# jinryan/RangeCLIP

Hardware: NVIDIA B200
Metric: pixel_text_infonce_fwd_bwd_throughput (higher is better)
Workload: dtype bf16

## Files before the change

include/rangeclip_b200.h:

```cpp
#ifndef RANGECLIP_B200_H_
#define RANGECLIP_B200_H_

#include <stdint.h>

#ifdef __cplusplus
extern "C" {
#endif

#define RC_ABI_VERSION 1

typedef enum { RC_F32 = 0, RC_BF16 = 1 } rc_dtype;

typedef enum {
  RC_OK = 0,
  RC_ERR_INVALID = -1,
  RC_ERR_UNSUPPORTED = -2,
  RC_ERR_CUDA = -3,
  RC_ERR_NO_DEVICE = -4
} rc_status;

int rc_abi_version(void);
const char* rc_last_error(void);
int64_t rc_launch_count(void);


int64_t rc_infonce_workspace_bytes(int B, int D, int64_t HW, int K, rc_dtype x_dtype);
int64_t rc_infonce_workspace_bytes_dt(int B, int D, int64_t HW, int K, rc_dtype x_dtype);

int rc_infonce_f32(const float* x, int B, int D, int64_t HW, int64_t ld_b,
                   const float* t, int K, const int32_t* y, const float* w, float inv_tau,
                   float* lse, double* loss_sum, double* w_sum,
                   const double* w_sum_in, const float* grad_scale,
                   float* dx, float* dt, double* dlogtau, void* stream);

#define RC_INFONCE_PREPASS_DONE 1
#define RC_INFONCE_KEEP_WEIGHT 2
#define RC_INFONCE_LSE_GIVEN 4
#define RC_INFONCE_TS_KERNEL 8
#define RC_INFONCE_ACCUMULATE_DX 16
int rc_infonce_bf16(const void* x, rc_dtype x_dtype, int B, int D, int64_t HW,
                    const void* t_bf16, const void* tt_bf16, int K,
                    const int32_t* y, const float* w, float inv_tau,
                    float* lse, double* loss_sum, double* w_sum,
                    const double* w_sum_in, const float* grad_scale,
                    void* dx, float* dt, double* dlogtau,
                    void* workspace, int64_t workspace_bytes, int flags, void* stream);
int rc_infonce_bf16_rep4(const void* x, rc_dtype x_dtype, int B, int D, int64_t HW,
                         const void* t_bf16, const void* tt_bf16, int K,
                         const int32_t* y4, const float* w4, float inv_tau,
                         float* lse, double* loss_sum, double* w_sum,
                         const double* w_sum_in, const float* grad_scale,
                         void* dx, float* dt, double* dlogtau,
                         void* workspace, int64_t workspace_bytes, int flags, void* stream);
int rc_infonce_bf16_kblocks(const void* x, rc_dtype x_dtype, int D, int64_t HW,
                            const void* t_bf16_all, const void* tt_bf16_all, int K, int n_blocks,
                            const int32_t* y_rel, const float* w_rep, float inv_tau,
                            float* lse, double* loss_sum, double* w_sum, const double* w_sum_in, const float* grad_scale,
                            void* dx_blocks, double* dlogtau, void* workspace, int64_t workspace_bytes, int flags, void* stream);
int rc_infonce_bf16_dyn(const void* x, rc_dtype x_dtype, int B, int D, int64_t HW,
                        const void* t_bf16, const void* tt_bf16, int K, const int32_t* k_dev,
                        const int32_t* y, const float* w, const float* log_tau_dev, int rep,
// ... 87 lines not shown
```

rangeclip_b200/csrc/infonce_ts.cu:

```cuda
#include "common.cuh"
#include "umma.cuh"
#include <float.h>
#include <stdlib.h>

namespace rc {
using namespace umma;

namespace ts {

#ifndef RC_TS_X_HINT
#define RC_TS_X_HINT 0
#endif

constexpr int kTilePx = 128;
constexpr int kThreads = 640;
constexpr int kXStages = 6;
constexpr int kTStages = 3;
constexpr int kStageBytes = 16 * 1024;
constexpr int kEpiBufs = 4;
constexpr int kEpiAhead = 2;
constexpr int kEpiBufBytes = 2048;
constexpr int kTmemCols = 512;
constexpr int kSlotCols = 256;
constexpr int kColAcc = 128, kAccCols = 64;
constexpr int kRegsCtl = 48, kRegsSoftmax = 120;
constexpr float kLog2e = 1.4426950408889634f;
constexpr float kLn2 = 0.6931471805599453f;

struct __align__(8) Bars {
  uint64_t xf[kXStages];
  uint64_t xfull[kXStages], xempty[kXStages];
  uint64_t tfull[kTStages], tempty[kTStages];
  uint64_t s_full[2], p_full[2];
  uint64_t acc_full[2][2], acc_empty[2][2];
  uint64_t sc_full[4];
  uint64_t ebar[8][kEpiBufs];
  uint32_t tmem_base, pad;
};

constexpr int kScaleBufs = 4;
constexpr int kOffT = kXStages * kStageBytes;
constexpr int kOffEpi = kOffT + kTStages * kStageBytes;
constexpr int kOffScale = kOffEpi + 8 * kEpiBufs * kEpiBufBytes;
constexpr int kOffXch = kOffScale + kScaleBufs * 128 * 4;
constexpr int kOffPart = kOffXch + 2 * 4 * 2 * 128 * 4;
constexpr int kOffBars = kOffPart + 8 * 128 * 4;
constexpr int kSmemBytes = kOffBars + (int)sizeof(Bars);
static_assert(kSmemBytes <= 232448, "shared-memory budget of one SM (227 KB)");

struct Params {
  int B, D, K, Kp;
  int64_t HW;
  int tiles_per_img, n_tiles, n_pairs;
  uint32_t tpi_magic;
  int keep_w;
  int acc_dx;
  const float* lse_in;
  int kb;
  const int32_t* y;
  const float* w;
  float inv_tau;
  const float* grad_scale;
  const double* w_sum_in;
  float* lse;
  double* loss_sum;
  double* w_sum;
  double* dlogtau;
};

__device__ __forceinline__ int div_tiles(const Params& prm, int tile) {
  int q = (int)__umulhi((uint32_t)tile, prm.tpi_magic);
  if (tile - q * prm.tiles_per_img >= prm.tiles_per_img) ++q;
  return q;
// ... 47 lines not shown
  const int n_clusters = gridDim.x / 2;
  const int cluster_id = blockIdx.x / 2;
  const int my_pairs = cluster_id < prm.n_pairs ? (prm.n_pairs - cluster_id + n_clusters - 1) / n_clusters : 0;

  if (threadIdx.x == 0) {
    tma_prefetch_desc(&map_x_s); tma_prefetch_desc(&map_t); tma_prefetch_desc(&map_tt);
    tma_prefetch_desc(&map_xe); tma_prefetch_desc(&map_dx);
    for (int i = 0; i < kXStages; ++i) { mbar_init(&bars->xf[i], 1); mbar_init(&bars->xfull[i], 2); mbar_init(&bars->xempty[i], 9); }
    for (int i = 0; i < kTStages; ++i) { mbar_init(&bars->tfull[i], 1); mbar_init(&bars->tempty[i], 1); }
    for (int sl = 0; sl < 2; ++sl) {
      mbar_init(&bars->s_full[sl], 1); mbar_init(&bars->p_full[sl], 16);
      for (int ab = 0; ab < 2; ++ab) { mbar_init(&bars->acc_full[sl][ab], 1); mbar_init(&bars->acc_empty[sl][ab], 16); }
    }
    for (int i = 0; i < kScaleBufs; ++i) mbar_init(&bars->sc_full[i], 4);
    for (int i = 0; i < 8; ++i)
      for (int j = 0; j < kEpiBufs; ++j) mbar_init(&bars->ebar[i][j], 1);
    fence_barrier_init();
  }
  if (warp == 2) tmem_alloc_2sm<kTmemCols>(&bars->tmem_base);
  tc_fence_before();
  cluster_sync();
  tc_fence_after();
  const uint32_t tmem = bars->tmem_base;
  const uint32_t idesc_s = make_idesc_bf16(256, prm.Kp,  1,  0);
  const uint32_t idesc_d = make_idesc_bf16(256, kAccCols, 0, 0);
  auto arrive_leader = [&](uint64_t* bar) {
    if (leader_cta) mbar_arrive(bar);
    else mbar_arrive_remote(map_to_cta(bar, 0));
  };
  auto arrive_leader_warp = [&](uint64_t* bar) {
    __syncwarp();
    if (elect_one()) arrive_leader(bar);
  };
  auto pair_of = [&](int l) -> int { return cluster_id + l * n_clusters; };
  auto koff_of = [&](int pj) -> int { return (kKB && prm.kb > 0) ? div_tiles(prm, 2 * pj) * 256 : 0; };

  if (warp < 4) {
    asm volatile("setmaxnreg.dec.sync.aligned.u32 %0;" ::"n"(kRegsCtl));
    if (warp == 0 && lane == 0) {
      uint32_t it = 0;
      auto load_s = [&](int l) {
        const int koff = koff_of(pair_of(l));
        for (int c = 0; c < n_dchunks; ++c, ++it) {
          const int st = it % kTStages;
          mbar_wait(&bars->tempty[st], ((it / kTStages) & 1) ^ 1, 1);
          if (leader_cta) mbar_arrive_expect_tx(&bars->tfull[st], 2 * Nh * 128);
          tma_load_2d_2sm(smem + kOffT + st * kStageBytes, &map_t, &bars->tfull[st], c * 64, koff + (int)rank * Nh);
        }
      };
      auto load_dx = [&](int l) {
        const int koff = koff_of(pair_of(l));
        for (int blk = 0; blk < n_blk; ++blk, ++it) {
          const int st = it % kTStages;
          mbar_wait(&bars->tempty[st], ((it / kTStages) & 1) ^ 1, 2);
          if (leader_cta) mbar_arrive_expect_tx(&bars->tfull[st], 2 * n_kchunks * 4096);
          for (int kc = 0; kc < n_kchunks; ++kc)
            tma_load_2d_2sm(smem + kOffT + st * kStageBytes + kc * 4096, &map_tt, &bars->tfull[st], koff + kc * 64,
                            blk * 64 + (int)rank * 32);
        }
      };
      if (my_pairs > 0) load_s(0);
      if (my_pairs > 1) load_s(1);
      for (int l = 0; l < my_pairs; ++l) {
        load_dx(l);
        if (l + 2 < my_pairs) load_s(l + 2);
      }
    } else if (warp == 3 && lane == 0) {
      uint32_t xit = 0;
      const uint64_t pol_keep = RC_TS_X_HINT ? l2_policy_evict_last() : 0;
      for (int l = 0; l < my_pairs; ++l) {
        int b, px0;
        tile_coords(prm, 2 * pair_of(l) + (int)rank, b, px0);
        for (int c = 0; c < n_dchunks; ++c, ++xit) {
          const int st = xit % kXStages;
          mbar_wait(&bars->xempty[st], ((xit / kXStages) & 1) ^ 1, 3);
          uint8_t* sb = smem + st * kStageBytes;
          mbar_arrive_expect_tx(&bars->xf[st], 2 * 8192);
          const int bx = (kKB && prm.kb > 0) ? (b < prm.B ? 0 : 1) : b;
          if (RC_TS_X_HINT) {
            tma_load_3d_hint(sb, &map_x_s, &bars->xf[st], px0, c * 64, bx, pol_keep);
            tma_load_3d_hint(sb + 8192, &map_x_s, &bars->xf[st], px0 + 64, c * 64, bx, pol_keep);
          } else {
            tma_load_3d(sb, &map_x_s, &bars->xf[st], px0, c * 64, bx);
            tma_load_3d(sb + 8192, &map_x_s, &bars->xf[st], px0 + 64, c * 64, bx);
          }
        }
      }
    } else if (warp == 1 && leader_cta) {
      uint32_t it = 0, xit = 0;
      uint32_t acc_uses[2][2] = {{0, 0}, {0, 0}};
      const uint32_t smem_base = smem_u32(smem);
      const uint64_t dsc_x = desc_mnmajor_sw128(0, 8192);
      const uint64_t dsc_k = desc_kmajor_sw128(0);
      auto wait_acc_free = [&](int sl, int ab) {
        mbar_wait(&bars->acc_empty[sl][ab], (acc_uses[sl][ab] & 1u) ^ 1u, 7);
      };
      auto issue_s = [&](int l) {
        const int sl = l & 1;
        const uint32_t s_tmem = tmem + sl * kSlotCols;
        wait_acc_free(sl, 0);
        wait_acc_free(sl, 1);
        tc_fence_after();
        for (int c = 0; c < n_dchunks; ++c, ++it, ++xit) {
          const int sa = xit % kXStages, sb_ = it % kTStages;
          mbar_wait(&bars->xfull[sa], (xit / kXStages) & 1, 5);
          mbar_wait(&bars->tfull[sb_], (it / kTStages) & 1, 6);
          tc_fence_after();
          const uint64_t xa = dsc_x + ((smem_base + sa * kStageBytes) >> 4);
          const uint64_t tb = dsc_k + ((smem_base + kOffT + sb_ * kStageBytes) >> 4);
          if (elect_one()) {
#pragma unroll
            for (int ks = 0; ks < 4; ++ks)
              mma_bf16_ss_2sm(s_tmem, xa + ((ks * 2048) >> 4), tb + ((ks * 32) >> 4), idesc_s, (c | ks) != 0);
            mma_commit_2sm(&bars->xempty[sa]);
            mma_commit_2sm(&bars->tempty[sb_]);
            if (c + 1 == n_dchunks) mma_commit_2sm(&bars->s_full[sl]);
          }
          __syncwarp();
        }
      };
      auto issue_dx = [&](int l) {
        const int sl = l & 1;
        const uint32_t base = tmem + sl * kSlotCols;
        mbar_wait(&bars->p_full[sl], (l >> 1) & 1, 9);
        tc_fence_after();
        for (int blk = 0; blk < n_blk; ++blk, ++it) {
          const int ab = blk & 1;
          wait_acc_free(sl, ab);
          const int st = it % kTStages;
          mbar_wait(&bars->tfull[st], (it / kTStages) & 1, 8);
          tc_fence_after();
          const uint64_t sb = dsc_k + ((smem_base + kOffT + st * kStageBytes) >> 4);
          const uint32_t dcol = base + kColAcc + ab * kAccCols;
          if (elect_one()) {
            for (int kc = 0; kc < n_kchunks; ++kc) {
#pragma unroll
              for (int ks = 0; ks < 4; ++ks)
                mma_bf16_ts_2sm(dcol, base + (kc * 4 + ks) * 8, sb + ((kc * 4096 + ks * 32) >> 4), idesc_d, (kc | ks) != 0);
            }
            mma_commit_2sm(&bars->tempty[st]);
            mma_commit_2sm(&bars->acc_full[sl][ab]);
          }
          __syncwarp();
          ++acc_uses[sl][ab];
        }
      };
      if (my_pairs > 0) issue_s(0);
      if (my_pairs > 1) issue_s(1);
      for (int l = 0; l < my_pairs; ++l) {
        issue_dx(l);
        if (l + 2 < my_pairs) issue_s(l + 2);
      }
    } else if (warp == 2 && lane == 0) {
      uint32_t xit = 0;
      for (int l = 0; l < my_pairs; ++l)
        for (int c = 0; c < n_dchunks; ++c, ++xit) {
          const int st = xit % kXStages;
          mbar_wait(&bars->xf[st], (xit / kXStages) & 1, 10);
          arrive_leader(&bars->xfull[st]);
        }
    }
  } else if (warp < 12) {
    asm volatile("setmaxnreg.inc.sync.aligned.u32 %0;" ::"n"(kRegsSoftmax));
    const int half = warp >= 8 ? 1 : 0;
    const int row = (warp & 3) * 32 + lane;
    const int Kh = prm.Kp >> 1;
    const int cb = half * Kh;
    const uint32_t lane_base = tmem + ((uint32_t)((warp & 3) * 32) << 16);
    float* xch_base = reinterpret_cast<float*>(smem + kOffXch);
    float loss_acc = 0.f, w_acc = 0.f, dlt_acc = 0.f;
    float inv_wsum = 0.f, gscale = 1.f;
    {
      const double ws = prm.w_sum_in[0];
      inv_wsum = ws > 0.0 ? (float)(1.0 / ws) : 0.f;
      if (prm.grad_scale) gscale = prm.grad_scale[0];
    }
    float nx_ok = 0.f, nx_w = 0.f;
    int nx_y = -1;
    auto load_pixel_scalars = [&](int l) {
      nx_ok = 0.f; nx_w = 0.f; nx_y = -1;
      if (l >= my_pairs) return;
      const int t = 2 * pair_of(l) + (int)rank;
      if (t < prm.n_tiles) {
        const int tb = div_tiles(prm, t);
        const int tpx = (t - tb * prm.tiles_per_img) * kTilePx + row;
        if (tpx < prm.HW) {
          const int64_t tm = (int64_t)tb * prm.HW + tpx;
          nx_ok = 1.f;
          if (R == 1) {
            nx_y = __ldg(prm.y + tm);
            nx_w = __ldg(prm.w + tm);
          } else {
            const int4 y4 = __ldg(reinterpret_cast<const int4*>(prm.y) + tm);
            nx_y = (y4.x & 255) | ((y4.y & 255) << 8) | ((y4.z & 255) << 16) | ((y4.w & 255) << 24);
          }
        }
      }
    };
    load_pixel_scalars(0);
    float* part_s = reinterpret_cast<float*>(smem + kOffPart);
    const int st_ = threadIdx.x - 128;
    const int ng = st_ & 15, nr = st_ >> 4;
    uint32_t nit = 0;
    auto norm_tile = [&]() -> float {
      float ss[8];
#pragma unroll
      for (int j = 0; j < 8; ++j) ss[j] = 0.f;
      for (int c = 0; c < n_dchunks; ++c, ++nit) {
        const int st = nit % kXStages;
        mbar_wait(&bars->xf[st], (nit / kXStages) & 1, 11);
        const uint8_t* base = smem + st * kStageBytes + (ng >> 3) * 8192 + nr * 128;
        const int ch = ng & 7;
#pragma unroll
        for (int rr = 0; rr < 4; ++rr) {
          const int rowd = nr + rr * 16;
          const uint4 v = *reinterpret_cast<const uint4*>(base + rr * 2048 + ((ch ^ (rowd & 7)) << 4));
          const uint32_t u[4] = {v.x, v.y, v.z, v.w};
#pragma unroll
          for (int j = 0; j < 4; ++j) {
            ss[2 * j] = sqacc_bf16x2_lo(ss[2 * j], u[j]);
            ss[2 * j + 1] = sqacc_bf16x2_hi(ss[2 * j + 1], u[j]);
          }
        }
        __syncwarp();
        if (elect_one()) mbar_arrive(&bars->xempty[st]);
      }
#pragma unroll
      for (int j = 0; j < 8; ++j) ss[j] += __shfl_xor_sync(0xffffffffu, ss[j], 16);
      if (lane < 16) {
        float4* dst = reinterpret_cast<float4*>(part_s + (warp - 4) * 128 + ng * 8);
        dst[0] = make_float4(ss[0], ss[1], ss[2], ss[3]);
        dst[1] = make_float4(ss[4], ss[5], ss[6], ss[7]);
      }
      named_bar_sync(5, 256);
      float q = 0.f;
#pragma unroll
      for (int wv = 0; wv < 8; ++wv) q += part_s[wv * 128 + row];
      return 1.f / fmaxf(sqrtf(q), 1e-12f);
    };
    const bool use_bound = prm.inv_tau * (2.02f * kLog2e) < 100.f;
    const float ml_bound = prm.inv_tau * (1.01f * kLog2e);
    for (int l = 0; l < my_pairs; ++l) {
      const int sl = l & 1;
      const int tile = 2 * pair_of(l) + (int)rank;
      const bool tile_ok = tile < prm.n_tiles;
      const int b = tile_ok ? div_tiles(prm, tile) : 0;
      const int px = tile_ok ? (tile - b * prm.tiles_per_img) * kTilePx + row : 0;
      const bool valid = tile_ok && px < prm.HW;
      const int64_t m = (int64_t)b * prm.HW + px;
      const int Kt = (kKB && prm.kb > 0) ? min(256, prm.K - 256 * b) : prm.K;
      const bool px_ok = nx_ok != 0.f;
      const int yi = nx_y;
      const float wi = (R == 1 && (yi >= 0 || (kKB && prm.keep_w))) ? nx_w : 0.f;
      load_pixel_scalars(l + 1);
      float* xch = xch_base + (l & 1) * (4 * 2 * 128);
      const uint32_t trow = lane_base + sl * kSlotCols + cb;
      const float inv_n_tile = norm_tile();
      const float inv_n = px_ok ? inv_n_tile : 0.f;
      const float zs = inv_n * prm.inv_tau;
      const float zl = zs * kLog2e;
      mbar_wait(&bars->s_full[sl], (l >> 1) & 1, 12);
      tc_fence_after();
      float ml = ml_bound;
      if (!use_bound) {
        float mx = -FLT_MAX;
        for (int c = 0; c * 32 < Kh; ++c) {
          const int nvalid = Kt - (cb + c * 32);
          if (nvalid <= 0) break;
          uint32_t r[32];
          tmem_ld_32x32(trow + c * 32, r);
          tmem_ld_wait();
#pragma unroll
          for (int i = 0; i < 32; ++i) if (i < nvalid) mx = fmaxf(mx, __uint_as_float(r[i]));
        }
        xch[(0 * 2 + half) * 128 + row] = mx;
        named_bar_sync(3, 256);
        mx = fmaxf(mx, xch[(0 * 2 + (half ^ 1)) * 128 + row]);
        ml = mx * zl;
      }
      uint32_t pk[64];
      float s0 = 0.f, s1 = 0.f, s2 = 0.f, s3 = 0.f, q0 = 0.f, q1 = 0.f, q2 = 0.f, q3 = 0.f;
      float sy[R];
#pragma unroll
      for (int j = 0; j < R; ++j) sy[j] = 0.f;
#pragma unroll
// ... 43 lines not shown
      } else {
        int4 y4 = make_int4(-1, -1, -1, -1);
        float4 w4 = make_float4(0.f, 0.f, 0.f, 0.f);
        if (px_ok) {
          y4 = __ldg(reinterpret_cast<const int4*>(prm.y) + m);
          w4 = __ldg(reinterpret_cast<const float4*>(prm.w) + m);
        }
        const int ya[4] = {y4.x, y4.y, y4.z, y4.w};
        const float wa[4] = {w4.x, w4.y, w4.z, w4.w};
#pragma unroll
        for (int j = 0; j < R; ++j) { yj[j] = ya[j]; wj[j] = ya[j] >= 0 ? wa[j] : 0.f; }
      }
      float wtot = 0.f, tz = 0.f;
      bool mine[R];
#pragma unroll
      for (int j = 0; j < R; ++j) {
        mine[j] = yj[j] >= cb && yj[j] < cb + Kh;
        wtot += wj[j];
        tz += mine[j] ? wj[j] * sy[j] : 0.f;
      }
      xch[(1 * 2 + half) * 128 + row] = sum;
      xch[(2 * 2 + half) * 128 + row] = sez;
      xch[(3 * 2 + half) * 128 + row] = tz;
      tc_fence_before();
      named_bar_sync(2, 256);
      tc_fence_after();
      sum += xch[(1 * 2 + (half ^ 1)) * 128 + row];
      sez += xch[(2 * 2 + (half ^ 1)) * 128 + row];
      tz += xch[(3 * 2 + (half ^ 1)) * 128 + row];
      if (kKB && prm.lse_in != nullptr && valid) sum = fast_exp2(fmaf(__ldg(prm.lse_in + (prm.kb > 0 ? (int64_t)px : m)), kLog2e, -ml));
      float lse = 0.f;
      if (half == 0) {
        lse = (ml + __log2f(sum)) * kLn2;
        loss_acc += wtot * lse - tz * zs;
        w_acc += wtot;
      }
      const float coefb = gscale * inv_wsum;
      const float coef = coefb * wtot;
      const float inv_sum = 1.f / sum;
      const float rsv = inv_n * prm.inv_tau * coef * inv_sum;
      if (half == 0) {
        const float cj = coef * sez * zs * inv_sum - coefb * tz * zs;
        sc_s[(l & (kScaleBufs - 1)) * 128 + row] = -(inv_n * inv_n * cj);
        dlt_acc -= cj;
        __syncwarp();
        if (lane == 0) mbar_arrive(&bars->sc_full[l & (kScaleBufs - 1)]);
      }
      {
        const uint32_t prow = lane_base + sl * kSlotCols + (cb >> 1);
        const uint32_t rs2 = pack_bf16x2(rsv, rsv);
        uint32_t g16[R];
        int grel[R];
#pragma unroll
        for (int j = 0; j < R; ++j) {
          grel[j] = -1;
          g16[j] = 0;
          if (mine[j]) {
            const float ey = fast_exp2(fmaf(sy[j], zl, -ml));
            float gv;
            if (R == 1) {
              gv = (ey - sum) * rsv;
            } else {
              float wk = 0.f;
#pragma unroll
              for (int i = 0; i < R; ++i) wk += (yj[i] == yj[j]) ? wj[i] : 0.f;
              gv = (ey - sum * (wtot > 0.f ? wk / wtot : 0.f)) * rsv;
            }
// ... 4 lines not shown
#pragma unroll
        for (int c = 0; c < 4; ++c) {
          if (c * 32 < Kh) {
            uint32_t v[16];
#pragma unroll
            for (int i = 0; i < 16; ++i) v[i] = bf2_mul(pk[c * 16 + i], rs2);
#pragma unroll
            for (int j = 0; j < R; ++j) {
              if (grel[j] >= 0 && (grel[j] >> 5) == c) {
                const int jj = (grel[j] >> 1) & 15;
                const bool hi = grel[j] & 1;
#pragma unroll
                for (int i = 0; i < 16; ++i)
                  if (i == jj) v[i] = hi ? ((v[i] & 0xffffu) | (g16[j] << 16)) : ((v[i] & 0xffff0000u) | g16[j]);
              }
            }
            tmem_st_32x16(prow + c * 16, v);
          }
        }
        tmem_st_wait();
        tc_fence_before();
        arrive_leader_warp(&bars->p_full[sl]);
      }
      if (half == 0 && valid && prm.lse && !(kKB && prm.lse_in != nullptr)) prm.lse[m] = lse;
    }
    if (half == 0) {
      loss_acc = warp_sum(loss_acc); w_acc = warp_sum(w_acc); dlt_acc = warp_sum(dlt_acc);
      if (lane == 0) {
        if (prm.loss_sum) atomicAdd(prm.loss_sum, (double)loss_acc);
        if (prm.w_sum) atomicAdd(prm.w_sum, (double)w_acc);
        if (prm.dlogtau) atomicAdd(prm.dlogtau, (double)dlt_acc);
      }
    }
  } else {
    const int ew = warp - 12;
    const int q = warp & 3, h = ew >> 2;
    uint8_t* ebuf = smem + kOffEpi + ew * (kEpiBufs * kEpiBufBytes);
    uint64_t* ebar = &bars->ebar[ew][0];
    const int total = my_pairs * n_blk;
    const uint64_t pol_first = l2_policy_evict_first();
    struct Cursor { int l, u, px, bo, bx; };
    auto cursor_pair = [&](Cursor& cu) {
      int b, px0;
      tile_coords(prm, 2 * pair_of(cu.l) + (int)rank, b, px0);
      cu.px = px0 + q * 32;
      cu.bo = b;
      cu.bx = (kKB && prm.kb > 0) ? (b < prm.B ? 0 : 1) : b;
    };
    auto cursor_next = [&](Cursor& cu) {
      if (++cu.u == n_blk) { cu.u = 0; ++cu.l; cursor_pair(cu); }
    };
    Cursor cs{0, 0, 0, 0, 0}, cr{0, 0, 0, 0, 0};
    cursor_pair(cs);
    cursor_pair(cr);
    int s_req = 0;
    auto request_x = [&]() {
      const int bi = s_req % kEpiBufs;
      mbar_arrive_expect_tx(&ebar[bi], kEpiBufBytes);
      tma_load_3d(ebuf + bi * kEpiBufBytes, &map_xe, &ebar[bi], cr.px, cr.u * 64 + h * 32, cr.bx);
    };
    for (; s_req < kEpiAhead && s_req < total; ++s_req) {
      if (lane == 0) request_x();
      cursor_next(cr);
    }
    const uint32_t moff = (uint32_t)((lane & 7) * 64 + ((((lane >> 3) ^ ((lane >> 1) & 3)) & 3) << 4));
    int s = 0;
    uint32_t acc_seen[2][2] = {{0, 0}, {0, 0}};
    for (int l = 0; l < my_pairs; ++l) {
      const int sl = l & 1;
      mbar_wait(&bars->sc_full[l & (kScaleBufs - 1)], (l >> 2) & 1, 14);
      uint32_t ncs2[4];
#pragma unroll
      for (int pb = 0; pb < 4; ++pb) {
        const float v = sc_s[(l & (kScaleBufs - 1)) * 128 + q * 32 + pb * 8 + (lane >> 2)];
        ncs2[pb] = pack_bf16x2(v, v);
      }
      const uint32_t tacc = tmem + ((uint32_t)(q * 32) << 16) + sl * kSlotCols + kColAcc + h * 32;
      for (int blk = 0; blk < n_blk; ++blk, ++s) {
        const int ab = blk & 1;
        mbar_wait(&bars->acc_full[sl][ab], acc_seen[sl][ab] & 1u, 15);
        ++acc_seen[sl][ab];
        tc_fence_after();
        uint32_t pa[4][4];
        {
          uint32_t r[16];
          tmem_ld_16x256b_x4(tacc + ab * kAccCols, r);
          tmem_ld_wait();
#pragma unroll
          for (int g = 0; g < 4; ++g) {
            pa[g][0] = pack_bf16x2(__uint_as_float(r[4 * g]), __uint_as_float(r[4 * g + 1]));
            pa[g][1] = pack_bf16x2(__uint_as_float(r[4 * g + 2]), __uint_as_float(r[4 * g + 3]));
          }
          tmem_ld_16x256b_x4(tacc + ab * kAccCols + (16u << 16), r);
          tmem_ld_wait();
#pragma unroll
          for (int g = 0; g < 4; ++g) {
            pa[g][2] = pack_bf16x2(__uint_as_float(r[4 * g]), __uint_as_float(r[4 * g + 1]));
            pa[g][3] = pack_bf16x2(__uint_as_float(r[4 * g + 2]), __uint_as_float(r[4 * g + 3]));
          }
        }
        tc_fence_before();
        arrive_leader_warp(&bars->acc_empty[sl][ab]);
        const int bi = s % kEpiBufs;
        mbar_wait(&ebar[bi], (s / kEpiBufs) & 1, 16);
        const uint32_t bx0 = smem_u32(ebuf + bi * kEpiBufBytes) + moff;
        uint32_t xm[4][4];
#pragma unroll
        for (int g = 0; g < 4; ++g) ldmatrix_x4_trans(bx0 + g * 512, xm[g]);
#pragma unroll
        for (int g = 0; g < 4; ++g) {
#pragma unroll
          for (int pb = 0; pb < 4; ++pb) xm[g][pb] = bf2_fma(ncs2[pb], xm[g][pb], pa[g][pb]);
          stmatrix_x4_trans(bx0 + g * 512, xm[g]);
        }
        fence_proxy_async_smem();
        __syncwarp();
        if (lane == 0) {
          if (kKB && prm.acc_dx) tma_reduce_add_3d(&map_dx, ebuf + bi * kEpiBufBytes, cs.px, cs.u * 64 + h * 32, cs.bo);
          else tma_store_3d_hint(&map_dx, ebuf + bi * kEpiBufBytes, cs.px, cs.u * 64 + h * 32, cs.bo, pol_first);
          tma_store_commit();
          if (s_req < total) {
            asm volatile("cp.async.bulk.wait_group.read %0;" ::"n"(kEpiBufs - kEpiAhead) : "memory");
            request_x();
          }
        }
        cursor_next(cs);
        if (s_req < total) { cursor_next(cr); ++s_req; }
        __syncwarp();
      }
    }
    if (lane == 0) tma_store_wait_all0();
  }
  tc_fence_before();
  cluster_sync();
  if (warp == 2) {
    tc_fence_after();
    tmem_dealloc_2sm<kTmemCols>(tmem);
  }
}

}

int launch_infonce_ts(const void* xsrc, void* dx, const void* t_bf16, const void* tt_bf16, int B, int D, int64_t HW, int K,
                      const int32_t* y, const float* w, float inv_tau, const float* grad_scale, const double* w_sum_in,
                      float* lse, double* loss_sum, double* w_sum, double* dlogtau, int rep, int keep_w, const float* lse_in,
                      int kb, int acc_dx, cudaStream_t s) {
  using namespace ts;
  const int Kp = kb > 0 ? 256 : (K + 63) / 64 * 64;
  const int Kall = kb > 0 ? kb * 256 : Kp;
  CUtensorMap m_xs, m_t, m_tt, m_xe, m_dx;
  int rcode;
  {
    const uint64_t dims[3] = {(uint64_t)HW, (uint64_t)D, (uint64_t)B};
    const uint64_t xdims[3] = {(uint64_t)HW, (uint64_t)D, (uint64_t)(kb > 0 ? 1 : B)};
    const uint64_t str[3] = {2, (uint64_t)HW * 2, (uint64_t)D * HW * 2};
    const uint32_t box_s[3] = {64, 64, 1};
    if ((rcode = make_tmap_bf16(&m_xs, xsrc, 3, xdims, str, box_s, "ts map_x_s"))) return rcode;
    const uint32_t box_o[3] = {32, 32, 1};
    if ((rcode = make_tmap_bf16(&m_xe, xsrc, 3, xdims, str, box_o, "ts map_xe"))) return rcode;
    if ((rcode = make_tmap_bf16(&m_dx, dx, 3, dims, str, box_o, "ts map_dx"))) return rcode;
    const uint64_t tdims[2] = {(uint64_t)D, (uint64_t)Kall}, tstr[2] = {2, (uint64_t)D * 2};
    const uint32_t tbox[2] = {64, (uint32_t)(Kp / 2)};
    if ((rcode = make_tmap_bf16(&m_t, t_bf16, 2, tdims, tstr, tbox, "ts map_t"))) return rcode;
    const uint64_t ttdims[2] = {(uint64_t)Kall, (uint64_t)D}, ttstr[2] = {2, (uint64_t)Kall * 2};
    const uint32_t ttbox[2] = {64, 32};
    if ((rcode = make_tmap_bf16(&m_tt, tt_bf16, 2, ttdims, ttstr, ttbox, "ts map_tt"))) return rcode;
  }
  Params prm;
  prm.B = B; prm.D = D; prm.K = K; prm.Kp = Kp; prm.HW = HW;
  prm.tiles_per_img = (int)((HW + kTilePx - 1) / kTilePx);
  if ((int64_t)B * prm.tiles_per_img > 0x3fffffff) return fail(RC_ERR_UNSUPPORTED, "rc_infonce_bf16: too many tiles");
  prm.n_tiles = B * prm.tiles_per_img;
  prm.tpi_magic = prm.tiles_per_img == 1 ? 0xffffffffu : (uint32_t)(0x100000000ull / (uint64_t)prm.tiles_per_img);
  prm.n_pairs = (prm.n_tiles + 1) / 2;
  prm.y = y; prm.w = w; prm.inv_tau = inv_tau; prm.grad_scale = grad_scale;
  prm.w_sum_in = w_sum_in; prm.lse = lse; prm.loss_sum = loss_sum; prm.w_sum = w_sum; prm.dlogtau = dlogtau;
  prm.keep_w = keep_w; prm.lse_in = lse_in; prm.kb = kb; prm.acc_dx = acc_dx;
  if (kb > 0 && (prm.tiles_per_img & 1)) return fail(RC_ERR_UNSUPPORTED, "rc_infonce_bf16_kblocks: HW must be a multiple of 256");
  int n_clusters = num_sms() / 2;
  if (n_clusters > prm.n_pairs) n_clusters = prm.n_pairs;
  const int grid = 2 * n_clusters;
  auto launch = [&](auto kernel) -> int {
    cudaError_t e = cudaFuncSetAttribute(kernel, cudaFuncAttributeMaxDynamicSharedMemorySize, kSmemBytes);
    if (e != cudaSuccess) return fail(RC_ERR_CUDA, "rc_infonce_bf16(ts): smem opt-in: %s", cudaGetErrorString(e));
    kernel<<<grid, kThreads, kSmemBytes, s>>>(m_xs, m_t, m_tt, m_xe, m_dx, prm);
    return check_launch("rc_infonce_bf16(ts)");
  };
  if (rep == 4) return launch(infonce_ts_kernel<4, false>);
  if (keep_w || lse_in != nullptr || kb > 0 || acc_dx) return launch(infonce_ts_kernel<1, true>);
  return launch(infonce_ts_kernel<1, false>);
}
// ... 89 lines not shown
```

rangeclip_b200/csrc/infonce_umma.cu:

```cuda
#include "common.cuh"
#include "umma.cuh"
#include <float.h>
#include <stdlib.h>

namespace rc {

using namespace umma;

PFN_encodeTiled get_encode_tiled() {
  static PFN_encodeTiled fn = nullptr;
  static bool tried = false;
  if (!tried) {
    tried = true;
    void* p = nullptr;
    cudaDriverEntryPointQueryResult qres;
    if (cudaGetDriverEntryPoint("cuTensorMapEncodeTiled", &p, cudaEnableDefault, &qres) == cudaSuccess &&
        qres == cudaDriverEntryPointSuccess)
      fn = (PFN_encodeTiled)p;
  }
  return fn;
}

int make_tmap_bf16(CUtensorMap* out, const void* base, int rank, const uint64_t* dims, const uint64_t* strides_bytes,
                   const uint32_t* box, const char* what) {
// ... 877 lines not shown
    RC_REQUIRE(!(flags & RC_INFONCE_LSE_GIVEN) || lse != nullptr, "rc_infonce_bf16: RC_INFONCE_LSE_GIVEN needs lse");
  }
  if (rep != 1) {
    if (!use_pair) return fail(RC_ERR_UNSUPPORTED, "rc_infonce_bf16_rep4: D=%d must be 256 or 512", D);
    RC_REQUIRE((reinterpret_cast<uintptr_t>(y) & 15) == 0 && (reinterpret_cast<uintptr_t>(w) & 15) == 0,
               "rc_infonce_bf16_rep4: y and w must be 16-byte aligned");
  }
  const bool skip_prepass = (flags & RC_INFONCE_PREPASS_DONE) || (use_pair && x_dtype == RC_BF16);
  if ((rcode = infonce_prepass_impl(x, x_dtype, B, D, HW, workspace, workspace_bytes, skip_prepass ? (cudaStream_t)-1 : s,
                                    &inv_norm, &xb))) return rcode;
  const void* xsrc = (x_dtype == RC_F32) ? (const void*)xb : x;
  if (dt != nullptr) {
    if (!use_pair || !bwd)
      return fail(RC_ERR_UNSUPPORTED, "rc_infonce_bf16: dText needs dx and D = 256 or 512 (use rc_infonce_f32 otherwise)");
    const int64_t base = rc_infonce_workspace_bytes(B, D, HW, K, x_dtype);
    RC_REQUIRE(workspace_bytes >= rc_infonce_workspace_bytes_dt(B, D, HW, K, x_dtype), "rc_infonce_bf16: workspace too small for dText");
    uint8_t* ws = reinterpret_cast<uint8_t*>((reinterpret_cast<uintptr_t>(workspace) + 255) & ~(uintptr_t)255);
    void* g = ws + ((base + 255) / 256) * 256;
    if ((rcode = launch_infonce_pair(xsrc, dx, t_bf16, tt_bf16, B, D, HW, K, inv_norm, y, w, inv_tau, grad_scale, w_sum_in, lse,
                                     loss_sum, w_sum, dlogtau, g, rep, 0, nullptr, 0, 0, k_dev, log_tau_dev, s))) return rcode;
    return launch_infonce_dt(g, xsrc, B, D, HW, K, dt, s);
  }
  if (use_pair) {
    if (bwd && (flags & RC_INFONCE_TS_KERNEL) && k_dev == nullptr && log_tau_dev == nullptr)
      return launch_infonce_ts(xsrc, dx, t_bf16, tt_bf16, B, D, HW, K, y, w, inv_tau, grad_scale, w_sum_in, lse, loss_sum, w_sum,
                               dlogtau, rep, keep_w, lse_in, 0, acc_dx, s);
    return launch_infonce_pair(xsrc, dx, t_bf16, tt_bf16, B, D, HW, K, inv_norm, y, w, inv_tau, grad_scale, w_sum_in, lse,
                               loss_sum, w_sum, dlogtau, nullptr, rep, keep_w, lse_in, 0, acc_dx, k_dev, log_tau_dev, s);
  }
  const int Kp = (K + 63) / 64 * 64;
  CUtensorMap m_xs, m_t, m_tt, m_xe, m_dx;
  {
    const uint64_t dims[3] = {(uint64_t)HW, (uint64_t)D, (uint64_t)B};
    const uint64_t str[3] = {2, (uint64_t)HW * 2, (uint64_t)D * HW * 2};
    const uint32_t box_s[3] = {64, 64, 1}, box_e[3] = {kStgPx, 128, 1};
    if ((rcode = make_tmap_bf16(&m_xs, xsrc, 3, dims, str, box_s, "map_x_s"))) return rcode;
    if ((rcode = make_tmap_bf16(&m_xe, xsrc, 3, dims, str, box_e, "map_x_e"))) return rcode;
    if ((rcode = make_tmap_bf16(&m_dx, bwd ? dx : xsrc, 3, dims, str, box_e, "map_dx"))) return rcode;
    const uint64_t tdims[2] = {(uint64_t)D, (uint64_t)Kp}, tstr[2] = {2, (uint64_t)D * 2};
    const uint32_t tbox[2] = {64, (uint32_t)Kp};
    if ((rcode = make_tmap_bf16(&m_t, t_bf16, 2, tdims, tstr, tbox, "map_t"))) return rcode;
    const uint64_t ttdims[2] = {(uint64_t)Kp, (uint64_t)D}, ttstr[2] = {2, (uint64_t)Kp * 2};
    const uint32_t ttbox[2] = {64, 128};
    if ((rcode = make_tmap_bf16(&m_tt, bwd ? tt_bf16 : t_bf16, 2, bwd ? ttdims : tdims, bwd ? ttstr : tstr,
                                bwd ? ttbox : tbox, "map_tt"))) return rcode;
  }
  InfoNceParams prm;
// ... 48 lines not shown

extern "C" int rc_infonce_bf16_kblocks(const void* x, rc_dtype x_dtype, int D, int64_t HW, const void* t_bf16_all,
                                       const void* tt_bf16_all, int K, int n_blocks, const int32_t* y_rel, const float* w_rep,
                                       float inv_tau, float* lse, double* loss_sum, double* w_sum, const double* w_sum_in,
                                       const float* grad_scale, void* dx_blocks, double* dlogtau, void* workspace,
                                       int64_t workspace_bytes, int flags, void* stream) {
  using namespace rc;
  RC_REQUIRE(x && t_bf16_all && y_rel && w_rep && workspace && lse, "rc_infonce_bf16_kblocks: null pointer");
  RC_REQUIRE(HW >= 0 && K >= 1 && n_blocks >= 1 && n_blocks == (K + 255) / 256, "rc_infonce_bf16_kblocks: n_blocks must be ceil(K / 256)");
  if (!infonce_pair_supported(D)) return fail(RC_ERR_UNSUPPORTED, "rc_infonce_bf16_kblocks: D=%d must be 256 or 512", D);
  if (HW % 256 != 0) return fail(RC_ERR_UNSUPPORTED, "rc_infonce_bf16_kblocks: HW=%lld must be a multiple of 256", (long long)HW);
  RC_REQUIRE((reinterpret_cast<uintptr_t>(t_bf16_all) & 15) == 0 && (reinterpret_cast<uintptr_t>(x) & 15) == 0, "rc_infonce_bf16_kblocks: alignment");
  const bool bwd = dx_blocks != nullptr;
  if (bwd) RC_REQUIRE(tt_bf16_all && w_sum_in && (flags & RC_INFONCE_LSE_GIVEN), "rc_infonce_bf16_kblocks: the backward needs tt_bf16_all, w_sum_in and RC_INFONCE_LSE_GIVEN");
  if (HW == 0) return RC_OK;
  int rcode = check_sm100("rc_infonce_bf16_kblocks");
  if (rcode) return rcode;
  cudaStream_t s = (cudaStream_t)stream;
  float* inv_norm; __nv_bfloat16* xb;
  const bool skip_prepass = (flags & RC_INFONCE_PREPASS_DONE) || x_dtype == RC_BF16;
  if ((rcode = infonce_prepass_impl(x, x_dtype, 1, D, HW, workspace, workspace_bytes, skip_prepass ? (cudaStream_t)-1 : s, &inv_norm, &xb))) return rcode;
  const void* xsrc = (x_dtype == RC_F32) ? (const void*)xb : x;
  const float* lse_in = (flags & RC_INFONCE_LSE_GIVEN) ? lse : nullptr;
  if (bwd && (flags & RC_INFONCE_TS_KERNEL))
    return launch_infonce_ts(xsrc, dx_blocks, t_bf16_all, tt_bf16_all, n_blocks, D, HW, K, y_rel, w_rep, inv_tau, grad_scale, w_sum_in,
                             lse, loss_sum, w_sum, dlogtau, 1, 1, lse_in, n_blocks, 0, s);
  return launch_infonce_pair(xsrc, dx_blocks, t_bf16_all, tt_bf16_all, n_blocks, D, HW, K, inv_norm, y_rel, w_rep, inv_tau, grad_scale,
                             w_sum_in, lse, loss_sum, w_sum, dlogtau, nullptr, 1, 1, lse_in, n_blocks, 0, nullptr, nullptr, s);
}

namespace rc {

__global__ void __cluster_dims__(2, 1, 1) __launch_bounds__(128, 1)
debug_umma_gemm_2sm_kernel(const __grid_constant__ CUtensorMap map_a, const __grid_constant__ CUtensorMap map_b, int N, int Kd,
                           float* __restrict__ c) {
  extern __shared__ __align__(1024) uint8_t smem[];
  uint8_t* sa = smem;
  uint8_t* sbm = smem + 16384;
  DebugBars* bars = reinterpret_cast<DebugBars*>(smem + 32768);
  const int warp = threadIdx.x >> 5, lane = threadIdx.x & 31;
  const uint32_t rank = cluster_ctarank();
  if (threadIdx.x == 0) {
    mbar_init(&bars->full, 1);
    mbar_init(&bars->done, 1);
    fence_barrier_init();
  }
  if (warp == 1) tmem_alloc_2sm<256>(&bars->tmem_base);
// ... 61 lines not shown
```

rangeclip_b200/ops.py:

```python
from __future__ import annotations

from typing import List, Optional, Sequence, Tuple

import torch

from . import _lib
from ._lib import RC_BF16, RC_F32, check

_I32_MAX = 2**31 - 1


def _need_cuda(*tensors: torch.Tensor) -> None:
    for t in tensors:
        if t is not None and not t.is_cuda:
            raise RuntimeError("rangeclip_b200 ops need CUDA tensors (no CPU fallback exists)")


def _p(t: Optional[torch.Tensor]):
    return None if t is None else t.data_ptr()


def _stream(t: torch.Tensor):
    return torch.cuda.current_stream(t.device).cuda_stream

# ... 202 lines not shown
                                        _p(gs), _p(dxb), acc[2:].data_ptr() if need_dx else None, _p(ws), ws_bytes, int(flags),
                                        st), "rc_infonce_bf16_dyn")
            dx = None
            if dxb is not None:
                dx = dxb.view(x.shape) if (x.dtype == torch.bfloat16 or keep_bf16) else scale_to(dxb.view(x.shape), x.dtype)
            return dict(loss_sum=acc[0], w_sum=acc[1], dlogtau=acc[2], lse=lse, dx=dx, dt=None, precision=precision, tv_sums=tv,
                        tv_codes=tv_codes)
        entry = L.rc_infonce_bf16 if rep == 1 else L.rc_infonce_bf16_rep4
        check(entry(_p(x), xdt, B, D, HW, _p(tb), _p(ttb), K, _p(y), _p(w), float(inv_tau), _p(lse),
                    acc[0:].data_ptr(), acc[1:].data_ptr(),
                    acc[3:].data_ptr() if need_grad else None, _p(gs), _p(dxb), _p(dt),
                    acc[2:].data_ptr() if need_dx else None, _p(ws), ws_bytes, int(flags), st),
              "rc_infonce_bf16" if rep == 1 else "rc_infonce_bf16_rep4")
        dx = None
        if dxb is not None:
            dx = dxb.view(x.shape) if (x.dtype == torch.bfloat16 or keep_bf16) else scale_to(dxb.view(x.shape), x.dtype)
    else:
        raise RuntimeError(f"infonce: unknown precision {precision!r}")
    return dict(loss_sum=acc[0], w_sum=acc[1], dlogtau=acc[2], lse=lse, dx=dx, dt=dt, precision=precision,
                tv_sums=tv if precision == "bf16" else None, tv_codes=tv_codes if precision == "bf16" else None)


RC_INFONCE_PREPASS_DONE, RC_INFONCE_KEEP_WEIGHT, RC_INFONCE_LSE_GIVEN, RC_INFONCE_TS_KERNEL, RC_INFONCE_ACCUMULATE_DX = 1, 2, 4, 8, 16


def kblocked_supported(D: int, HW: int) -> bool:
    return D in (256, 512) and HW % 8 == 0 and HW > 0


def infonce_kblocked_raw(x: torch.Tensor, t_norm: torch.Tensor, y: torch.Tensor, w: torch.Tensor, inv_tau: float,
                         need_dx: bool, block: int = 256, keep_bf16: bool = False):
    _need_cuda(x, t_norm, y, w)
    x, B, D, HW = _emb3(x)
    if not kblocked_supported(D, HW):
        raise RuntimeError(f"infonce_kblocked: needs D in (256, 512) and HW % 8 == 0; got D={D}, HW={HW}")
    K = t_norm.shape[0]
    M = B * HW
    dev = x.device
    y = y.reshape(-1).to(torch.int32)
    w = (w.reshape(-1).to(torch.float32) * (y >= 0)).contiguous()
    L = _lib.lib()
    st = _stream(x)
    xdt = _dt(x)
    ws_bytes = int(L.rc_infonce_workspace_bytes(B, D, HW, block, xdt))
    ws = torch.empty(ws_bytes, device=dev, dtype=torch.uint8)
    if x.dtype != torch.bfloat16:
# ... 882 lines not shown
```

Baseline: 1756.

## Default to TS kernel, reschedule S/dX issue order, enable X cache hint

```diff
diff --git a/include/rangeclip_b200.h b/include/rangeclip_b200.h
--- a/include/rangeclip_b200.h
+++ b/include/rangeclip_b200.h
@@ -37,6 +37,7 @@
 #define RC_INFONCE_KEEP_WEIGHT 2
 #define RC_INFONCE_LSE_GIVEN 4
 #define RC_INFONCE_TS_KERNEL 8
+#define RC_INFONCE_SS_KERNEL 32
 #define RC_INFONCE_ACCUMULATE_DX 16
 int rc_infonce_bf16(const void* x, rc_dtype x_dtype, int B, int D, int64_t HW,
                     const void* t_bf16, const void* tt_bf16, int K,
diff --git a/rangeclip_b200/csrc/infonce_ts.cu b/rangeclip_b200/csrc/infonce_ts.cu
--- a/rangeclip_b200/csrc/infonce_ts.cu
+++ b/rangeclip_b200/csrc/infonce_ts.cu
@@ -9,7 +9,25 @@
 namespace ts {
 
 #ifndef RC_TS_X_HINT
-#define RC_TS_X_HINT 0
+#define RC_TS_X_HINT 1
+#endif
+
+#ifdef RC_TIMING
+__device__ __forceinline__ unsigned long long globaltimer_ns() {
+  unsigned long long t;
+  asm volatile("mov.u64 %0, %%globaltimer;" : "=l"(t));
+  return t;
+}
+#define RC_T0(name) const long long name = clock64()
+#define RC_TACC(idx, name) wt[idx] += clock64() - name
+#define RC_WAIT(fn, bar, par, tag) do { const long long t0_ = clock64(); fn(bar, par, tag); wt[tag] += clock64() - t0_; } while (0)
+#define RC_EV(iter, id) do { if (prm.dbg != nullptr && blockIdx.x < 2 && lane == 0 && (iter) >= 40u && (iter) < 44u) \
+    prm.dbg[256 + blockIdx.x * 192 + ((iter) - 40u) * 48 + (id)] = (long long)globaltimer_ns(); } while (0)
+#else
+#define RC_T0(name)
+#define RC_TACC(idx, name)
+#define RC_WAIT(fn, bar, par, tag) fn(bar, par, tag)
+#define RC_EV(iter, id)
 #endif
 
 constexpr int kTilePx = 128;
@@ -23,6 +41,7 @@
 constexpr int kTmemCols = 512;
 constexpr int kSlotCols = 256;
 constexpr int kColAcc = 128, kAccCols = 64;
+constexpr int kDxLead = 2;
 constexpr int kRegsCtl = 48, kRegsSoftmax = 120;
 constexpr float kLog2e = 1.4426950408889634f;
 constexpr float kLn2 = 0.6931471805599453f;
@@ -44,11 +63,14 @@
 constexpr int kOffScale = kOffEpi + 8 * kEpiBufs * kEpiBufBytes;
 constexpr int kOffXch = kOffScale + kScaleBufs * 128 * 4;
 constexpr int kOffPart = kOffXch + 2 * 4 * 2 * 128 * 4;
-constexpr int kOffBars = kOffPart + 8 * 128 * 4;
+constexpr int kOffAcc = kOffPart + 8 * 128 * 4;
+constexpr int kOffBars = kOffAcc + 3 * 128 * 4;
 constexpr int kSmemBytes = kOffBars + (int)sizeof(Bars);
 static_assert(kSmemBytes <= 232448, "shared-memory budget of one SM (227 KB)");
 
 struct Params {
+  long long* dbg;
+  int ablate;
   int B, D, K, Kp;
   int64_t HW;
   int tiles_per_img, n_tiles, n_pairs;
@@ -142,6 +164,12 @@
   cluster_sync();
   tc_fence_after();
   const uint32_t tmem = bars->tmem_base;
+#ifdef RC_TIMING
+  long long wt[16];
+#pragma unroll
+  for (int i = 0; i < 16; ++i) wt[i] = 0;
+  const long long t_start = clock64();
+#endif
   const uint32_t idesc_s = make_idesc_bf16(256, prm.Kp,  1,  0);
   const uint32_t idesc_d = make_idesc_bf16(256, kAccCols, 0, 0);
   auto arrive_leader = [&](uint64_t* bar) {
@@ -163,16 +191,24 @@
         const int koff = koff_of(pair_of(l));
         for (int c = 0; c < n_dchunks; ++c, ++it) {
           const int st = it % kTStages;
-          mbar_wait(&bars->tempty[st], ((it / kTStages) & 1) ^ 1, 1);
+          RC_WAIT(mbar_wait, &bars->tempty[st], ((it / kTStages) & 1) ^ 1, 1);
+          if ((prm.ablate & 256) && it >= (uint32_t)kTStages) {
+            if (leader_cta) mbar_arrive(&bars->tfull[st]);
+            continue;
+          }
           if (leader_cta) mbar_arrive_expect_tx(&bars->tfull[st], 2 * Nh * 128);
           tma_load_2d_2sm(smem + kOffT + st * kStageBytes, &map_t, &bars->tfull[st], c * 64, koff + (int)rank * Nh);
         }
       };
-      auto load_dx = [&](int l) {
+      auto load_dx = [&](int l, int b0, int b1) {
         const int koff = koff_of(pair_of(l));
-        for (int blk = 0; blk < n_blk; ++blk, ++it) {
+        for (int blk = b0; blk < b1; ++blk, ++it) {
           const int st = it % kTStages;
-          mbar_wait(&bars->tempty[st], ((it / kTStages) & 1) ^ 1, 2);
+          RC_WAIT(mbar_wait, &bars->tempty[st], ((it / kTStages) & 1) ^ 1, 2);
+          if ((prm.ablate & 256) && it >= (uint32_t)kTStages) {
+            if (leader_cta) mbar_arrive(&bars->tfull[st]);
+            continue;
+          }
           if (leader_cta) mbar_arrive_expect_tx(&bars->tfull[st], 2 * n_kchunks * 4096);
           for (int kc = 0; kc < n_kchunks; ++kc)
             tma_load_2d_2sm(smem + kOffT + st * kStageBytes + kc * 4096, &map_tt, &bars->tfull[st], koff + kc * 64,
@@ -180,10 +216,10 @@
         }
       };
       if (my_pairs > 0) load_s(0);
-      if (my_pairs > 1) load_s(1);
       for (int l = 0; l < my_pairs; ++l) {
-        load_dx(l);
-        if (l + 2 < my_pairs) load_s(l + 2);
+        load_dx(l, 0, kDxLead);
+        if (l + 1 < my_pairs) load_s(l + 1);
+        load_dx(l, kDxLead, n_blk);
       }
     } else if (warp == 3 && lane == 0) {
       uint32_t xit = 0;
@@ -193,7 +229,7 @@
         tile_coords(prm, 2 * pair_of(l) + (int)rank, b, px0);
         for (int c = 0; c < n_dchunks; ++c, ++xit) {
           const int st = xit % kXStages;
-          mbar_wait(&bars->xempty[st], ((xit / kXStages) & 1) ^ 1, 3);
+          RC_WAIT(mbar_wait, &bars->xempty[st], ((xit / kXStages) & 1) ^ 1, 3);
           uint8_t* sb = smem + st * kStageBytes;
           mbar_arrive_expect_tx(&bars->xf[st], 2 * 8192);
           const int bx = (kKB && prm.kb > 0) ? (b < prm.B ? 0 : 1) : b;
@@ -208,23 +244,24 @@
       }
     } else if (warp == 1 && leader_cta) {
       uint32_t it = 0, xit = 0;
-      uint32_t acc_uses[2][2] = {{0, 0}, {0, 0}};
+      uint32_t acc_par = 0;
       const uint32_t smem_base = smem_u32(smem);
       const uint64_t dsc_x = desc_mnmajor_sw128(0, 8192);
       const uint64_t dsc_k = desc_kmajor_sw128(0);
-      auto wait_acc_free = [&](int sl, int ab) {
-        mbar_wait(&bars->acc_empty[sl][ab], (acc_uses[sl][ab] & 1u) ^ 1u, 7);
+      auto wait_acc_free = [&](int sl, int ab, int tag) {
+        RC_WAIT(mbar_wait, &bars->acc_empty[sl][ab], ((acc_par >> (2 * sl + ab)) & 1u) ^ 1u, tag);
       };
       auto issue_s = [&](int l) {
         const int sl = l & 1;
         const uint32_t s_tmem = tmem + sl * kSlotCols;
-        wait_acc_free(sl, 0);
-        wait_acc_free(sl, 1);
+        wait_acc_free(sl, 0, 7);
+        wait_acc_free(sl, 1, 7);
         tc_fence_after();
+        RC_EV(l, 0);
         for (int c = 0; c < n_dchunks; ++c, ++it, ++xit) {
           const int sa = xit % kXStages, sb_ = it % kTStages;
-          mbar_wait(&bars->xfull[sa], (xit / kXStages) & 1, 5);
-          mbar_wait(&bars->tfull[sb_], (it / kTStages) & 1, 6);
+          RC_WAIT(mbar_wait, &bars->xfull[sa], (xit / kXStages) & 1, 5);
+          RC_WAIT(mbar_wait, &bars->tfull[sb_], (it / kTStages) & 1, 6);
           tc_fence_after();
           const uint64_t xa = dsc_x + ((smem_base + sa * kStageBytes) >> 4);
           const uint64_t tb = dsc_k + ((smem_base + kOffT + sb_ * kStageBytes) >> 4);
@@ -238,17 +275,22 @@
           }
           __syncwarp();
         }
+        RC_EV(l, 1);
       };
-      auto issue_dx = [&](int l) {
+      auto issue_dx = [&](int l, int b0, int b1) {
         const int sl = l & 1;
         const uint32_t base = tmem + sl * kSlotCols;
-        mbar_wait(&bars->p_full[sl], (l >> 1) & 1, 9);
-        tc_fence_after();
-        for (int blk = 0; blk < n_blk; ++blk, ++it) {
+        if (b0 == 0) {
+          RC_WAIT(mbar_wait, &bars->p_full[sl], (l >> 1) & 1, 9);
+          tc_fence_after();
+          RC_EV(l, 2);
+        }
+        for (int blk = b0; blk < b1; ++blk, ++it) {
           const int ab = blk & 1;
-          wait_acc_free(sl, ab);
+          wait_acc_free(sl, ab, 4);
+          if (blk < 8) RC_EV(l, 3 + blk);
           const int st = it % kTStages;
-          mbar_wait(&bars->tfull[st], (it / kTStages) & 1, 8);
+          RC_WAIT(mbar_wait, &bars->tfull[st], (it / kTStages) & 1, 8);
           tc_fence_after();
           const uint64_t sb = dsc_k + ((smem_base + kOffT + st * kStageBytes) >> 4);
           const uint32_t dcol = base + kColAcc + ab * kAccCols;
@@ -262,14 +304,15 @@
             mma_commit_2sm(&bars->acc_full[sl][ab]);
           }
           __syncwarp();
-          ++acc_uses[sl][ab];
-        }
+          acc_par ^= 1u << (2 * sl + ab);
+        }
+        if (b1 == n_blk) RC_EV(l, 11);
       };
       if (my_pairs > 0) issue_s(0);
-      if (my_pairs > 1) issue_s(1);
       for (int l = 0; l < my_pairs; ++l) {
-        issue_dx(l);
-        if (l + 2 < my_pairs) issue_s(l + 2);
+        issue_dx(l, 0, kDxLead);
+        if (l + 1 < my_pairs) issue_s(l + 1);
+        issue_dx(l, kDxLead, n_blk);
       }
     } else if (warp == 2 && lane == 0) {
       uint32_t xit = 0;
@@ -288,12 +331,12 @@
     const int cb = half * Kh;
     const uint32_t lane_base = tmem + ((uint32_t)((warp & 3) * 32) << 16);
     float* xch_base = reinterpret_cast<float*>(smem + kOffXch);
-    float loss_acc = 0.f, w_acc = 0.f, dlt_acc = 0.f;
-    float inv_wsum = 0.f, gscale = 1.f;
+    float* acc_s = reinterpret_cast<float*>(smem + kOffAcc) + row;
+    if (half == 0) acc_s[0] = acc_s[128] = acc_s[256] = 0.f;
+    float coefb;
     {
       const double ws = prm.w_sum_in[0];
-      inv_wsum = ws > 0.0 ? (float)(1.0 / ws) : 0.f;
-      if (prm.grad_scale) gscale = prm.grad_scale[0];
+      coefb = (prm.grad_scale ? prm.grad_scale[0] : 1.f) * (ws > 0.0 ? (float)(1.0 / ws) : 0.f);
     }
     float nx_ok = 0.f, nx_w = 0.f;
     int nx_y = -1;
@@ -328,7 +371,7 @@
       for (int j = 0; j < 8; ++j) ss[j] = 0.f;
       for (int c = 0; c < n_dchunks; ++c, ++nit) {
         const int st = nit % kXStages;
-        mbar_wait(&bars->xf[st], (nit / kXStages) & 1, 11);
+        RC_WAIT(mbar_wait, &bars->xf[st], (nit / kXStages) & 1, 11);
         const uint8_t* base = smem + st * kStageBytes + (ng >> 3) * 8192 + nr * 128;
         const int ch = ng & 7;
 #pragma unroll
@@ -375,12 +418,17 @@
       load_pixel_scalars(l + 1);
       float* xch = xch_base + (l & 1) * (4 * 2 * 128);
       const uint32_t trow = lane_base + sl * kSlotCols + cb;
+      RC_T0(tnorm);
       const float inv_n_tile = norm_tile();
+      RC_TACC(1, tnorm);
+      if (warp == 4) RC_EV(l, 12);
       const float inv_n = px_ok ? inv_n_tile : 0.f;
       const float zs = inv_n * prm.inv_tau;
       const float zl = zs * kLog2e;
-      mbar_wait(&bars->s_full[sl], (l >> 1) & 1, 12);
+      RC_WAIT(mbar_wait, &bars->s_full[sl], (l >> 1) & 1, 12);
       tc_fence_after();
+      if (warp == 4) RC_EV(l, 13);
+      RC_T0(texp);
       float ml = ml_bound;
       if (!use_bound) {
         float mx = -FLT_MAX;
@@ -470,9 +518,14 @@
       xch[(1 * 2 + half) * 128 + row] = sum;
       xch[(2 * 2 + half) * 128 + row] = sez;
       xch[(3 * 2 + half) * 128 + row] = tz;
+      RC_TACC(2, texp);
+      if (warp == 4) RC_EV(l, 14);
       tc_fence_before();
+      RC_T0(txch);
       named_bar_sync(2, 256);
+      RC_TACC(13, txch);
       tc_fence_after();
+      RC_T0(tpst);
       sum += xch[(1 * 2 + (half ^ 1)) * 128 + row];
       sez += xch[(2 * 2 + (half ^ 1)) * 128 + row];
       tz += xch[(3 * 2 + (half ^ 1)) * 128 + row];
@@ -480,17 +533,16 @@
       float lse = 0.f;
       if (half == 0) {
         lse = (ml + __log2f(sum)) * kLn2;
-        loss_acc += wtot * lse - tz * zs;
-        w_acc += wtot;
-      }
-      const float coefb = gscale * inv_wsum;
+        acc_s[0] += wtot * lse - tz * zs;
+        acc_s[128] += wtot;
+      }
       const float coef = coefb * wtot;
       const float inv_sum = 1.f / sum;
       const float rsv = inv_n * prm.inv_tau * coef * inv_sum;
       if (half == 0) {
         const float cj = coef * sez * zs * inv_sum - coefb * tz * zs;
         sc_s[(l & (kScaleBufs - 1)) * 128 + row] = -(inv_n * inv_n * cj);
-        dlt_acc -= cj;
+        acc_s[256] -= cj;
         __syncwarp();
         if (lane == 0) mbar_arrive(&bars->sc_full[l & (kScaleBufs - 1)]);
       }
@@ -541,10 +593,12 @@
         tc_fence_before();
         arrive_leader_warp(&bars->p_full[sl]);
       }
+      RC_TACC(3, tpst);
+      if (warp == 4) RC_EV(l, 15);
       if (half == 0 && valid && prm.lse && !(kKB && prm.lse_in != nullptr)) prm.lse[m] = lse;
     }
     if (half == 0) {
-      loss_acc = warp_sum(loss_acc); w_acc = warp_sum(w_acc); dlt_acc = warp_sum(dlt_acc);
+      const float loss_acc = warp_sum(acc_s[0]), w_acc = warp_sum(acc_s[128]), dlt_acc = warp_sum(acc_s[256]);
       if (lane == 0) {
         if (prm.loss_sum) atomicAdd(prm.loss_sum, (double)loss_acc);
         if (prm.w_sum) atomicAdd(prm.w_sum, (double)w_acc);
@@ -575,8 +629,13 @@
     int s_req = 0;
     auto request_x = [&]() {
       const int bi = s_req % kEpiBufs;
+      if (prm.ablate & 1) {
+        mbar_arrive(&ebar[bi]);
+        return;
+      }
       mbar_arrive_expect_tx(&ebar[bi], kEpiBufBytes);
-      tma_load_3d(ebuf + bi * kEpiBufBytes, &map_xe, &ebar[bi], cr.px, cr.u * 64 + h * 32, cr.bx);
+      if (RC_TS_X_HINT) tma_load_3d_hint(ebuf + bi * kEpiBufBytes, &map_xe, &ebar[bi], cr.px, cr.u * 64 + h * 32, cr.bx, pol_first);
+      else tma_load_3d(ebuf + bi * kEpiBufBytes, &map_xe, &ebar[bi], cr.px, cr.u * 64 + h * 32, cr.bx);
     };
     for (; s_req < kEpiAhead && s_req < total; ++s_req) {
       if (lane == 0) request_x();
@@ -584,10 +643,10 @@
     }
     const uint32_t moff = (uint32_t)((lane & 7) * 64 + ((((lane >> 3) ^ ((lane >> 1) & 3)) & 3) << 4));
     int s = 0;
-    uint32_t acc_seen[2][2] = {{0, 0}, {0, 0}};
+    uint32_t acc_par = 0;
     for (int l = 0; l < my_pairs; ++l) {
       const int sl = l & 1;
-      mbar_wait(&bars->sc_full[l & (kScaleBufs - 1)], (l >> 2) & 1, 14);
+      RC_WAIT(mbar_wait, &bars->sc_full[l & (kScaleBufs - 1)], (l >> 2) & 1, 14);
       uint32_t ncs2[4];
 #pragma unroll
       for (int pb = 0; pb < 4; ++pb) {
@@ -597,9 +656,11 @@
       const uint32_t tacc = tmem + ((uint32_t)(q * 32) << 16) + sl * kSlotCols + kColAcc + h * 32;
       for (int blk = 0; blk < n_blk; ++blk, ++s) {
         const int ab = blk & 1;
-        mbar_wait(&bars->acc_full[sl][ab], acc_seen[sl][ab] & 1u, 15);
-        ++acc_seen[sl][ab];
+        RC_WAIT(mbar_wait, &bars->acc_full[sl][ab], (acc_par >> (2 * sl + ab)) & 1u, 15);
+        acc_par ^= 1u << (2 * sl + ab);
         tc_fence_after();
+        if (warp == 12 && blk < 8) RC_EV(l, 20 + 2 * blk);
+        RC_T0(tld);
         uint32_t pa[4][4];
         {
           uint32_t r[16];
@@ -620,8 +681,10 @@
         }
         tc_fence_before();
         arrive_leader_warp(&bars->acc_empty[sl][ab]);
+        RC_TACC(3, tld);
         const int bi = s % kEpiBufs;
-        mbar_wait(&ebar[bi], (s / kEpiBufs) & 1, 16);
+        RC_WAIT(mbar_wait, &ebar[bi], (s / kEpiBufs) & 1, 4);
+        RC_T0(tmath);
         const uint32_t bx0 = smem_u32(ebuf + bi * kEpiBufBytes) + moff;
         uint32_t xm[4][4];
 #pragma unroll
@@ -634,22 +697,36 @@
         }
         fence_proxy_async_smem();
         __syncwarp();
+        RC_TACC(2, tmath);
         if (lane == 0) {
-          if (kKB && prm.acc_dx) tma_reduce_add_3d(&map_dx, ebuf + bi * kEpiBufBytes, cs.px, cs.u * 64 + h * 32, cs.bo);
-          else tma_store_3d_hint(&map_dx, ebuf + bi * kEpiBufBytes, cs.px, cs.u * 64 + h * 32, cs.bo, pol_first);
-          tma_store_commit();
+          if (!(prm.ablate & 2)) {
+            if (kKB && prm.acc_dx) tma_reduce_add_3d(&map_dx, ebuf + bi * kEpiBufBytes, cs.px, cs.u * 64 + h * 32, cs.bo);
+            else tma_store_3d_hint(&map_dx, ebuf + bi * kEpiBufBytes, cs.px, cs.u * 64 + h * 32, cs.bo, pol_first);
+            tma_store_commit();
+          }
           if (s_req < total) {
+            RC_T0(tsw);
             asm volatile("cp.async.bulk.wait_group.read %0;" ::"n"(kEpiBufs - kEpiAhead) : "memory");
+            RC_TACC(5, tsw);
             request_x();
           }
         }
         cursor_next(cs);
         if (s_req < total) { cursor_next(cr); ++s_req; }
         __syncwarp();
+        if (warp == 12 && blk < 8) RC_EV(l, 21 + 2 * blk);
       }
     }
     if (lane == 0) tma_store_wait_all0();
   }
+#ifdef RC_TIMING
+  if (prm.dbg != nullptr && blockIdx.x < 2 && lane == 0 && (warp <= 1 || warp == 3 || warp == 4 || warp == 12)) {
+    wt[0] = clock64() - t_start;
+    const int role = warp == 0 ? 0 : (warp == 1 ? 1 : (warp == 4 ? 2 : (warp == 12 ? 3 : 4)));
+#pragma unroll
+    for (int i = 0; i < 16; ++i) prm.dbg[(blockIdx.x * 5 + role) * 16 + i] = wt[i];
+  }
+#endif
   tc_fence_before();
   cluster_sync();
   if (warp == 2) {
@@ -686,6 +763,11 @@
     if ((rcode = make_tmap_bf16(&m_tt, tt_bf16, 2, ttdims, ttstr, ttbox, "ts map_tt"))) return rcode;
   }
   Params prm;
+  prm.dbg = debug_timing_buffer();
+  prm.ablate = 0;
+#ifdef RC_BRINGUP
+  { const char* ab = getenv("RANGECLIP_B200_ABLATE"); prm.ablate = ab ? atoi(ab) : 0; }
+#endif
   prm.B = B; prm.D = D; prm.K = K; prm.Kp = Kp; prm.HW = HW;
   prm.tiles_per_img = (int)((HW + kTilePx - 1) / kTilePx);
   if ((int64_t)B * prm.tiles_per_img > 0x3fffffff) return fail(RC_ERR_UNSUPPORTED, "rc_infonce_bf16: too many tiles");
diff --git a/rangeclip_b200/csrc/infonce_umma.cu b/rangeclip_b200/csrc/infonce_umma.cu
--- a/rangeclip_b200/csrc/infonce_umma.cu
+++ b/rangeclip_b200/csrc/infonce_umma.cu
@@ -923,7 +923,7 @@
     return launch_infonce_dt(g, xsrc, B, D, HW, K, dt, s);
   }
   if (use_pair) {
-    if (bwd && (flags & RC_INFONCE_TS_KERNEL) && k_dev == nullptr && log_tau_dev == nullptr)
+    if (bwd && !(flags & RC_INFONCE_SS_KERNEL) && k_dev == nullptr && log_tau_dev == nullptr)
       return launch_infonce_ts(xsrc, dx, t_bf16, tt_bf16, B, D, HW, K, y, w, inv_tau, grad_scale, w_sum_in, lse, loss_sum, w_sum,
                                dlogtau, rep, keep_w, lse_in, 0, acc_dx, s);
     return launch_infonce_pair(xsrc, dx, t_bf16, tt_bf16, B, D, HW, K, inv_norm, y, w, inv_tau, grad_scale, w_sum_in, lse,
@@ -1018,7 +1018,7 @@
   if ((rcode = infonce_prepass_impl(x, x_dtype, 1, D, HW, workspace, workspace_bytes, skip_prepass ? (cudaStream_t)-1 : s, &inv_norm, &xb))) return rcode;
   const void* xsrc = (x_dtype == RC_F32) ? (const void*)xb : x;
   const float* lse_in = (flags & RC_INFONCE_LSE_GIVEN) ? lse : nullptr;
-  if (bwd && (flags & RC_INFONCE_TS_KERNEL))
+  if (bwd && !(flags & RC_INFONCE_SS_KERNEL))
     return launch_infonce_ts(xsrc, dx_blocks, t_bf16_all, tt_bf16_all, n_blocks, D, HW, K, y_rel, w_rep, inv_tau, grad_scale, w_sum_in,
                              lse, loss_sum, w_sum, dlogtau, 1, 1, lse_in, n_blocks, 0, s);
   return launch_infonce_pair(xsrc, dx_blocks, t_bf16_all, tt_bf16_all, n_blocks, D, HW, K, inv_norm, y_rel, w_rep, inv_tau, grad_scale,
diff --git a/rangeclip_b200/ops.py b/rangeclip_b200/ops.py
--- a/rangeclip_b200/ops.py
+++ b/rangeclip_b200/ops.py
@@ -248,6 +248,7 @@
 
 
 RC_INFONCE_PREPASS_DONE, RC_INFONCE_KEEP_WEIGHT, RC_INFONCE_LSE_GIVEN, RC_INFONCE_TS_KERNEL, RC_INFONCE_ACCUMULATE_DX = 1, 2, 4, 8, 16
+RC_INFONCE_SS_KERNEL = 32
 
 
 def kblocked_supported(D: int, HW: int) -> bool:
```

New measurement: 1889 (median of 6 runs). 7.6% higher.
